# lucidrains/progen

Hardware: NVIDIA H100
Metric: tokens_per_sec (higher is better)
Workload: dtype bf16

## Files before the change

include/progen_b200.h:

```cpp
#ifndef PROGEN_B200_H
#define PROGEN_B200_H
#include <stdint.h>

#ifdef __cplusplus
extern "C" {
#endif

#define PROGEN_F32 0
#define PROGEN_BF16 1

#define PROGEN_BACKEND_SIMT 0
#define PROGEN_BACKEND_TC 1

#define PROGEN_EPI_STORE 0
#define PROGEN_EPI_ROTARY 1
#define PROGEN_EPI_RESIDUAL 2
#define PROGEN_EPI_GLU 3
#define PROGEN_EPI_GELU 4
#define PROGEN_EPI_GLU_BWD 5
#define PROGEN_EPI_GELU_BWD 6
#define PROGEN_EPI_ACCUM 7

const char* progen_version(void);
const char* progen_last_error(void);
// ... 1 lines not shown
long long progen_launch_count(void);

typedef struct progen_gemm_t {
  int32_t M, N, K;
  int32_t a_mn_major, b_mn_major;
  int32_t batch;
  int32_t batch_reduce;
  int32_t causal;
  int32_t split_k;
  int32_t in_dtype, out_dtype, epi_kind, backend;
  int32_t seq_len, dim_head;
  int32_t atomic, tril, tril_rows;
  int64_t lda, ldb;
  int64_t a_batch_rows, b_batch_rows, d_batch_rows;
  int64_t ldo, ldo2, ldaux;
  const void* A;
  const void* B;
  void* out;
  void* out2;
  const float* bias;
  const void* aux;
  const float* rot_sin;
  const float* rot_cos;
} progen_gemm_t;

int progen_gemm(const progen_gemm_t* desc, void* stream);

int progen_embed_fwd(const int* tokens, const float* table, float* x, long long T, int d, int V, void* stream);
int progen_embed_bwd(const int* tokens, const float* dx, float* dtable, long long T, int d, int V, void* stream);

int progen_ln_shift_fwd(const void* x, long long ldx, int x_dtype, const float* scale, void* y, long long ldy, int y_dtype,
                        float* mean, float* rstd, long long T, int d, int seq_len, int shift, void* stream);
int progen_ln_shift_bwd(const void* dy, long long lddy, int act_dtype, const void* x, long long ldx, int x_dtype,
                        const float* scale, const float* mean, const float* rstd, float* dres, void* dout, long long ldo,
                        float* dscale, float* dres_colsum, long long T, int d, int seq_len, int shift, int residual,
                        void* stream);

int progen_colsum(const void* in, long long ld, int dtype, float* out, long long T, int N, void* stream);

int progen_ce_fwd_bwd(const void* logits, int dtype, const int* labels, float* weights, float* loss, void* dlogits,
                      int dlogits_dtype, int B, int n, int V, float inv_batch, void* stream);

int progen_token_logprob(const void* logits, int dtype, const int* labels, float* logp, float* seq_ll, float* seq_count,
                         int B, int n, int V, void* stream);
int progen_preference_head(const void* logits, int dtype, const int* labels, const float* ref_ll, float* logp, float* seq_ll,
                           float* seq_count, float* weights, float* stats, float* loss, float* ce_scratch, void* dlogits,
// ... 124 lines not shown
```

progen_b200/csrc/api.cu:

```cuda
#include <stdarg.h>
#include "gemm.h"
#include "../../include/progen_b200.h"

static thread_local char g_err[1024] = "";
unsigned long long g_progen_launches = 0;

void progen_set_error(const char* fmt, ...) {
  va_list ap;
  va_start(ap, fmt);
  vsnprintf(g_err, sizeof(g_err), fmt, ap);
  va_end(ap);
}

extern "C" {

const char* progen_version(void) { return "progen_b200 0.1.0 (sm_90a; wgmma/TMA GEMM, CUDA " CUDA_VERSION_STR ")"; }

const char* progen_last_error(void) { return g_err; }

long long progen_launch_count(void) { return (long long)__atomic_load_n(&g_progen_launches, __ATOMIC_RELAXED); }

int progen_device_check(void) {
  int dev = 0;
  PG_CUDA(cudaGetDevice(&dev));
// ... 2 lines not shown
  if (prop.major != 9) {
    progen_set_error("device %d (%s) is sm_%d%d; libprogen_b200 is built for sm_90a only", dev, prop.name, prop.major,
                     prop.minor);
    return PROGEN_ERR_DEVICE;
  }
  return PROGEN_OK;
}

int progen_gemm(const progen_gemm_t* d, void* stream) {
  PG_CHECK_ARG(d != nullptr);
  GemmArgs g;
  g.M = d->M; g.N = d->N; g.K = d->K;
  g.A = d->A; g.lda = d->lda; g.a_mn_major = d->a_mn_major;
  g.B = d->B; g.ldb = d->ldb; g.b_mn_major = d->b_mn_major;
  g.batch = d->batch < 1 ? 1 : d->batch;
  g.a_batch_rows = d->a_batch_rows; g.b_batch_rows = d->b_batch_rows; g.d_batch_rows = d->d_batch_rows;
  g.batch_reduce = d->batch_reduce; g.causal = d->causal; g.split_k = d->split_k < 1 ? 1 : d->split_k;
  g.in_dtype = d->in_dtype; g.out_dtype = d->out_dtype; g.epi_kind = d->epi_kind;
  g.epi.out = d->out; g.epi.ldo = d->ldo; g.epi.out2 = d->out2; g.epi.ldo2 = d->ldo2;
  g.epi.bias = d->bias; g.epi.aux = d->aux; g.epi.ldaux = d->ldaux;
  g.epi.rot_sin = d->rot_sin; g.epi.rot_cos = d->rot_cos;
  g.epi.seq_len = d->seq_len > 0 ? d->seq_len : 1; g.epi.dim_head = d->dim_head > 0 ? d->dim_head : 2;
  g.epi.atomic = d->atomic; g.epi.tril = d->tril; g.epi.tril_rows = d->tril_rows > 0 ? d->tril_rows : 1;
  PG_CHECK_ARG(g.epi_kind >= 0 && g.epi_kind < EPI_NUM_KINDS);
  PG_CHECK_ARG(g.epi.out != nullptr);
  if (g.epi_kind == EPI_GLU || g.epi_kind == EPI_GELU) PG_CHECK_ARG(g.epi.bias != nullptr);
  if (g.epi_kind == EPI_GLU_BWD || g.epi_kind == EPI_GELU_BWD) PG_CHECK_ARG(g.epi.aux != nullptr);
  if (g.epi_kind == EPI_ROTARY) PG_CHECK_ARG(g.epi.rot_sin && g.epi.rot_cos && d->seq_len > 0 && d->dim_head > 0 && d->dim_head % 2 == 0);
  if (d->backend == PROGEN_BACKEND_TC) return gemm_tc_launch(g, (cudaStream_t)stream);
  if (d->backend == PROGEN_BACKEND_SIMT) return gemm_simt_launch(g, (cudaStream_t)stream);
  progen_set_error("progen_gemm: unknown backend %d", d->backend);
  return PROGEN_ERR_ARG;
}

}
```

progen_b200/csrc/epilogues.cuh:

```cuda
#pragma once
#include "common.cuh"

enum EpiKind : int {
  EPI_STORE = 0,
  EPI_ROTARY = 1,
  EPI_RESIDUAL = 2,
  EPI_GLU = 3,
  EPI_GELU = 4,
  EPI_GLU_BWD = 5,
  EPI_GELU_BWD = 6,
  EPI_ACCUM = 7,
  EPI_NUM_KINDS = 8
};

struct EpiArgs {
  void* out; long long ldo;
  void* out2; long long ldo2;
  const float* bias;
  const void* aux; long long ldaux;
  const float* rot_sin;
  const float* rot_cos;
  int seq_len; int dim_head;
  int atomic;
  int tril;
  int tril_rows;
};

struct DirectIO {
  template <int N, typename T> __device__ __forceinline__ void store(T* p, long long, const float (&v)[N], bool valid) const {
    if (valid) store_vec<N>(p, v);
  }
  template <int N, typename T> __device__ __forceinline__ void load(const T* p, long long, float (&v)[N], bool valid) const {
    if (valid) load_vec<N>(p, v);
    else {
#pragma unroll
      for (int i = 0; i < N; ++i) v[i] = 0.f;
    }
  }
};

template <int NV> __device__ __forceinline__ void add_bias(const float* __restrict__ bias, int col, float (&v)[NV]) {
#pragma unroll
  for (int i = 0; i < NV; i += 4) {
    const float4 b = __ldg(reinterpret_cast<const float4*>(bias + col + i));
    v[i] += b.x; v[i + 1] += b.y; v[i + 2] += b.z; v[i + 3] += b.w;
  }
}

template <int KIND, typename TO, int NV, typename IO>
__device__ __forceinline__ void epi_apply(const EpiArgs& e, const IO& io, long long row, int col, float (&v)[NV], bool valid) {
  constexpr bool FAST = sizeof(TO) == 2;
  if constexpr (KIND == EPI_STORE) {
    if (e.bias) add_bias<NV>(e.bias, col, v);
    io.template store<NV>(reinterpret_cast<TO*>(e.out) + row * e.ldo + col, e.ldo, v, valid);
  } else if constexpr (KIND == EPI_ROTARY) {
    const int pos = (int)(row % e.seq_len);
    const int half = e.dim_head >> 1;
    const float* sp = e.rot_sin + (long long)pos * half;
    const float* cp = e.rot_cos + (long long)pos * half;
    float o[NV];
    if (e.dim_head % NV == 0) {
      const int j0 = (col % e.dim_head) >> 1;
      float s[NV / 2], c[NV / 2];
      if constexpr (NV >= 32) {
        io.template load<NV / 2>(sp + j0, half, s, true);
        io.template load<NV / 2>(cp + j0, half, c, true);
      } else {
        load_vec<NV / 2>(sp + j0, s);
        load_vec<NV / 2>(cp + j0, c);
      }
#pragma unroll
      for (int i = 0; i < NV; i += 2) {
        o[i] = v[i] * c[i >> 1] - v[i + 1] * s[i >> 1];
        o[i + 1] = v[i + 1] * c[i >> 1] + v[i] * s[i >> 1];
      }
    } else {
#pragma unroll
      for (int i = 0; i < NV; i += 2) {
        const int j = ((col + i) % e.dim_head) >> 1;
        const float s = __ldg(sp + j), c = __ldg(cp + j);
        o[i] = v[i] * c - v[i + 1] * s;
        o[i + 1] = v[i + 1] * c + v[i] * s;
      }
    }
    io.template store<NV>(reinterpret_cast<TO*>(e.out) + row * e.ldo + col, e.ldo, o, valid);
  } else if constexpr (KIND == EPI_RESIDUAL) {
    float* p = reinterpret_cast<float*>(e.out) + row * e.ldo + col;
    float r[NV];
    if (e.aux) io.template load<NV>(reinterpret_cast<const float*>(e.aux) + row * e.ldaux + col, e.ldaux, r, valid);
    else io.template load<NV>(const_cast<const float*>(p), e.ldo, r, valid);
    if (e.bias) add_bias<NV>(e.bias, col, v);
#pragma unroll
    for (int i = 0; i < NV; ++i) r[i] += v[i];
    io.template store<NV>(p, e.ldo, r, valid);
  } else if constexpr (KIND == EPI_GLU) {
    add_bias<NV>(e.bias, col, v);
    if (e.out2) io.template store<NV>(reinterpret_cast<TO*>(e.out2) + row * e.ldo2 + col, e.ldo2, v, valid);
    TO* po = reinterpret_cast<TO*>(e.out) + row * e.ldo + (col >> 1);
    if constexpr (NV >= 16) {
      float o[NV / 2];
#pragma unroll
      for (int i = 0; i < NV / 2; ++i) o[i] = v[2 * i] * gelu_fwd<FAST>(v[2 * i + 1]);
      io.template store<NV / 2>(po, e.ldo, o, valid);
    } else {
      if (valid) {
#pragma unroll
        for (int i = 0; i < NV / 2; ++i) po[i] = from_f32<TO>(v[2 * i] * gelu_fwd<FAST>(v[2 * i + 1]));
      }
    }
  } else if constexpr (KIND == EPI_GELU) {
    add_bias<NV>(e.bias, col, v);
    if (e.out2) io.template store<NV>(reinterpret_cast<TO*>(e.out2) + row * e.ldo2 + col, e.ldo2, v, valid);
    float o[NV];
#pragma unroll
    for (int i = 0; i < NV; ++i) o[i] = gelu_fwd<FAST>(v[i]);
    io.template store<NV>(reinterpret_cast<TO*>(e.out) + row * e.ldo + col, e.ldo, o, valid);
  } else if constexpr (KIND == EPI_GLU_BWD) {
    float u[2 * NV];
    io.template load<2 * NV>(reinterpret_cast<const TO*>(e.aux) + row * e.ldaux + 2 * col, e.ldaux, u, valid);
#pragma unroll
    for (int i = 0; i < NV; ++i) {
      const float dh = v[i], val = u[2 * i], gate = u[2 * i + 1];
      float gf, gd;
      gelu_fwd_bwd<FAST>(gate, gf, gd);
      u[2 * i] = dh * gf;
      u[2 * i + 1] = dh * val * gd;
    }
    io.template store<2 * NV>(reinterpret_cast<TO*>(e.out) + row * e.ldo + 2 * col, e.ldo, u, valid);
  } else if constexpr (KIND == EPI_GELU_BWD) {
    float u[NV];
    io.template load<NV>(reinterpret_cast<const TO*>(e.aux) + row * e.ldaux + col, e.ldaux, u, valid);
#pragma unroll
    for (int i = 0; i < NV; ++i) v[i] *= gelu_bwd<FAST>(u[i]);
    io.template store<NV>(reinterpret_cast<TO*>(e.out) + row * e.ldo + col, e.ldo, v, valid);
  } else if constexpr (KIND == EPI_ACCUM) {
    if (!valid) return;
    float* p = reinterpret_cast<float*>(e.out) + row * e.ldo + col;
    const int lim = e.tril ? (int)(row % e.tril_rows) : 0x7fffffff;
    if (e.atomic) {
#pragma unroll
      for (int i = 0; i < NV; i += 4) {
        if (col + i + 3 <= lim) {
          asm volatile("red.global.add.v4.f32 [%0], {%1, %2, %3, %4};" ::"l"(p + i), "f"(v[i]), "f"(v[i + 1]),
                       "f"(v[i + 2]), "f"(v[i + 3]) : "memory");
        } else {
#pragma unroll
          for (int j = 0; j < 4; ++j)
            if (col + i + j <= lim) atomicAdd(p + i + j, v[i + j]);
        }
      }
    } else {
      float r[NV];
      load_vec<NV>(p, r);
#pragma unroll
      for (int i = 0; i < NV; ++i) r[i] += (col + i <= lim) ? v[i] : 0.f;
      store_vec<NV>(p, r);
    }
  }
}
```

progen_b200/csrc/gemm_simt.cu:

```cuda
#include "gemm.h"

namespace {

constexpr int SBM = 128, SBN = 128, SBK = 16;

struct SimtDev {
  int M, N, K;
  long long a_rs, a_cs, b_rs, b_cs;
  long long a_bs, b_bs;
  long long d_batch_rows;
  int batch_reduce, causal;
  EpiArgs epi;
};

template <typename TI, int KIND, typename TO>
__global__ void __launch_bounds__(256) gemm_simt_kernel(const TI* __restrict__ A, const TI* __restrict__ B, const SimtDev g) {
  __shared__ float As[SBK][SBM + 4];
  __shared__ float Bs[SBK][SBN + 4];
  const int z = blockIdx.z;
  const int m0 = blockIdx.y * SBM, n0 = blockIdx.x * SBN;
  const TI* Ab = A + (long long)z * g.a_bs;
  const TI* Bb = B + (long long)z * g.b_bs;
  const int tid = threadIdx.x;
  const int tx = tid & 15, ty = tid >> 4;
// ... 25 lines not shown
      const int gn = n0 + n, gk = k0 + k;
      Bs[k][n] = (gn < g.N && gk < k_end) ? to_f32(Bb[gn * g.b_rs + gk * g.b_cs]) : 0.f;
    }
    __syncthreads();
#pragma unroll
    for (int k = 0; k < SBK; ++k) {
      float a[8], b[8];
      const float4 a0 = *reinterpret_cast<const float4*>(&As[k][ty * 8]);
      const float4 a1 = *reinterpret_cast<const float4*>(&As[k][ty * 8 + 4]);
      const float4 b0 = *reinterpret_cast<const float4*>(&Bs[k][tx * 8]);
      const float4 b1 = *reinterpret_cast<const float4*>(&Bs[k][tx * 8 + 4]);
      a[0] = a0.x; a[1] = a0.y; a[2] = a0.z; a[3] = a0.w; a[4] = a1.x; a[5] = a1.y; a[6] = a1.z; a[7] = a1.w;
      b[0] = b0.x; b[1] = b0.y; b[2] = b0.z; b[3] = b0.w; b[4] = b1.x; b[5] = b1.y; b[6] = b1.z; b[7] = b1.w;
#pragma unroll
      for (int i = 0; i < 8; ++i)
#pragma unroll
        for (int j = 0; j < 8; ++j) acc[i][j] = fmaf(a[i], b[j], acc[i][j]);
    }
    __syncthreads();
  }

  const int col = n0 + tx * 8;
  if (col >= g.N) return;
#pragma unroll
  for (int i = 0; i < 8; ++i) {
    const int m = m0 + ty * 8 + i;
    if (m >= g.M) break;
    const long long row = (g.batch_reduce ? 0 : (long long)z * g.d_batch_rows) + m;
    epi_apply<KIND, TO, 8>(g.epi, DirectIO{}, row, col, acc[i], true);
  }
}

template <typename TI, int KIND, typename TO>
int launch(const GemmArgs& a, const SimtDev& gd, cudaStream_t stream) {
  dim3 grid((a.N + SBN - 1) / SBN, (a.M + SBM - 1) / SBM, a.batch);
  gemm_simt_kernel<TI, KIND, TO><<<grid, 256, 0, stream>>>(reinterpret_cast<const TI*>(a.A),
                                                          reinterpret_cast<const TI*>(a.B), gd);
  PG_LAUNCH_CHECK();
  return PROGEN_OK;
}

template <typename TI, typename TO>
int dispatch_kind(const GemmArgs& a, const SimtDev& gd, cudaStream_t s) {
  switch (a.epi_kind) {
    case EPI_STORE: return launch<TI, EPI_STORE, TO>(a, gd, s);
    case EPI_ROTARY: return launch<TI, EPI_ROTARY, TO>(a, gd, s);
    case EPI_RESIDUAL: return launch<TI, EPI_RESIDUAL, float>(a, gd, s);
    case EPI_GLU: return launch<TI, EPI_GLU, TO>(a, gd, s);
    case EPI_GELU: return launch<TI, EPI_GELU, TO>(a, gd, s);
    case EPI_GLU_BWD: return launch<TI, EPI_GLU_BWD, TO>(a, gd, s);
    case EPI_GELU_BWD: return launch<TI, EPI_GELU_BWD, TO>(a, gd, s);
    case EPI_ACCUM: return launch<TI, EPI_ACCUM, float>(a, gd, s);
    default: break;
  }
  progen_set_error("gemm_simt: unknown epilogue %d", a.epi_kind);
  return PROGEN_ERR_UNSUPPORTED;
}

}

int gemm_simt_launch(const GemmArgs& a, cudaStream_t stream) {
  PG_CHECK_ARG(a.M > 0 && a.N > 0 && a.K > 0 && a.batch >= 1);
  PG_CHECK_ARG(a.N % 8 == 0);
  PG_CHECK_ARG(a.split_k == 1);
  PG_CHECK_ARG(!a.batch_reduce || (a.epi_kind == EPI_ACCUM && a.epi.atomic));
  SimtDev gd;
  gd.M = a.M; gd.N = a.N; gd.K = a.K;
  gd.a_rs = a.a_mn_major ? 1 : a.lda; gd.a_cs = a.a_mn_major ? a.lda : 1;
  gd.b_rs = a.b_mn_major ? 1 : a.ldb; gd.b_cs = a.b_mn_major ? a.ldb : 1;
  gd.a_bs = a.a_batch_rows * a.lda; gd.b_bs = a.b_batch_rows * a.ldb;
  gd.d_batch_rows = a.d_batch_rows;
  gd.batch_reduce = a.batch_reduce; gd.causal = a.causal;
  gd.epi = a.epi;
  if (a.in_dtype == PG_F32) {
    return dispatch_kind<float, float>(a, gd, stream);
  }
  if (a.out_dtype == PG_BF16) return dispatch_kind<bf16, bf16>(a, gd, stream);
  return dispatch_kind<bf16, float>(a, gd, stream);
}
```

progen_b200/csrc/gemm_tc.cu:

```cuda
#include <cuda.h>
#include <algorithm>
#include <mutex>
#include <unordered_map>
#include "gemm.h"
#include "tc_ptx.cuh"

namespace {

using namespace tc;

constexpr int BM = 128;
constexpr int BN = 128;
constexpr int BK = 64;
constexpr int WG_K = 16;
constexpr int THREADS = 384;
constexpr int A_BYTES = BM * BK * 2;
constexpr int B_BYTES = BN * BK * 2;
constexpr int STAGE_BYTES = A_BYTES + B_BYTES;
constexpr int STAGES = 4;
constexpr int EPI_ROWS = 64;
constexpr int CS_LD = BN + 4;
constexpr int CS_BYTES = EPI_ROWS * CS_LD * 4;
constexpr int SMEM_TOTAL = 1024  + STAGES * STAGE_BYTES + 2 * CS_BYTES + 2 * STAGES * 8;
static_assert(SMEM_TOTAL <= 227 * 1024, "H100: 227 KiB of shared memory per block");
constexpr int BAR_TURN = 1, BAR_EPI = 3;
constexpr int PRODUCER_REGS = 40, CONSUMER_REGS = 232;
static_assert(128 * PRODUCER_REGS + 256 * CONSUMER_REGS <= 65536, "register file");

__device__ __forceinline__ void named_bar_sync(int id, int n) { asm volatile("bar.sync %0, %1;" ::"r"(id), "r"(n) : "memory"); }
__device__ __forceinline__ void named_bar_arrive(int id, int n) { asm volatile("bar.arrive %0, %1;" ::"r"(id), "r"(n) : "memory"); }
template <int R> __device__ __forceinline__ void setmaxnreg_dec() { asm volatile("setmaxnreg.dec.sync.aligned.u32 %0;" ::"n"(R)); }
template <int R> __device__ __forceinline__ void setmaxnreg_inc() { asm volatile("setmaxnreg.inc.sync.aligned.u32 %0;" ::"n"(R)); }

struct GemmDev {
  int M, N, K;
  int batch, batch_reduce;
  int a_batch_rows, b_batch_rows;
  long long d_batch_rows;
  int causal, split_k;
  EpiArgs epi;
};

struct TileInfo {
// ... 109 lines not shown
    for (int kb = ti.kb_begin; kb < ti.kb_end; ++kb) {
      mbar_wait(full_bar(stage), phase);
      const uint32_t sa = smem_base + stage * STAGE_BYTES;
      const uint64_t adesc0 = make_smem_desc<A_MN>(sa), adesc1 = make_smem_desc<A_MN>(sa + 8192);
      const uint64_t bdesc = make_smem_desc<B_MN>(sa + A_BYTES);
      constexpr uint32_t a_step = A_MN ? (2048 >> 4) : (32 >> 4), b_step = B_MN ? (2048 >> 4) : (32 >> 4);
      fence_regs(acc[0]);
      fence_regs(acc[1]);
      wgmma_fence();
#pragma unroll
      for (int k = 0; k < BK / WG_K; ++k) {
        wgmma_m64n128k16_bf16<A_MN ? 1 : 0, B_MN ? 1 : 0>(acc[0], adesc0 + (uint64_t)(k * a_step), bdesc + (uint64_t)(k * b_step));
        wgmma_m64n128k16_bf16<A_MN ? 1 : 0, B_MN ? 1 : 0>(acc[1], adesc1 + (uint64_t)(k * a_step), bdesc + (uint64_t)(k * b_step));
      }
      wgmma_commit();
      fence_regs(acc[0]);
      fence_regs(acc[1]);
      wgmma_wait<1>();
      if (prev >= 0 && tid == 0) mbar_arrive(empty_bar(prev));
      prev = stage;
      advance(1);
    }
    if (t + (int)gridDim.x < tiles) named_bar_arrive(BAR_TURN + (c ^ 1), 256);
    wgmma_wait<0>();
    fence_regs(acc[0]);
    fence_regs(acc[1]);
    if (prev >= 0 && tid == 0) mbar_arrive(empty_bar(prev));

    const int w = tid >> 5, lane = tid & 31;
    const int r0 = 16 * w + (lane >> 2), c0 = 2 * (lane & 3);
#pragma unroll
    for (int h = 0; h < 2; ++h) {
      named_bar_sync(BAR_EPI + c, 128);
#pragma unroll
      for (int j = 0; j < BN / 8; ++j) {
        *reinterpret_cast<float2*>(cs + r0 * CS_LD + 8 * j + c0) = make_float2(acc[h][4 * j], acc[h][4 * j + 1]);
        *reinterpret_cast<float2*>(cs + (r0 + 8) * CS_LD + 8 * j + c0) = make_float2(acc[h][4 * j + 2], acc[h][4 * j + 3]);
      }
      named_bar_sync(BAR_EPI + c, 128);
#pragma unroll 1
      for (int idx = tid; idx < EPI_ROWS * (BN / 8); idx += 128) {
        const int r = idx / (BN / 8), cc = (idx % (BN / 8)) * 8;
        const int m = ti.m0 + EPI_ROWS * h + r, col = ti.n0 + cc;
        if (m >= g.M || col >= g.N) continue;
        float v[8];
        const float4 x0 = *reinterpret_cast<const float4*>(cs + r * CS_LD + cc);
        const float4 x1 = *reinterpret_cast<const float4*>(cs + r * CS_LD + cc + 4);
        v[0] = x0.x; v[1] = x0.y; v[2] = x0.z; v[3] = x0.w; v[4] = x1.x; v[5] = x1.y; v[6] = x1.z; v[7] = x1.w;
        const long long row = (g.batch_reduce ? 0 : (long long)ti.z * g.d_batch_rows) + m;
        epi_apply<KIND, TO, 8>(g.epi, DirectIO{}, row, col, v, true);
      }
    }
  }
}

typedef CUresult (*EncodeTiledFn)(CUtensorMap*, CUtensorMapDataType, cuuint32_t, void*, const cuuint64_t*,
                                  const cuuint64_t*, const cuuint32_t*, const cuuint32_t*, CUtensorMapInterleave,
                                  CUtensorMapSwizzle, CUtensorMapL2promotion, CUtensorMapFloatOOBfill);

EncodeTiledFn get_encode_fn() {
  static EncodeTiledFn fn = nullptr;
  static std::once_flag once;
  std::call_once(once, [] {
    void* p = nullptr;
    cudaDriverEntryPointQueryResult q;
    if (cudaGetDriverEntryPoint("cuTensorMapEncodeTiled", &p, cudaEnableDefault, &q) == cudaSuccess &&
        q == cudaDriverEntryPointSuccess)
      fn = reinterpret_cast<EncodeTiledFn>(p);
  });
  return fn;
}

struct MapKey {
// ... 54 lines not shown
    attr_set = true;
  }
  kern<<<std::min(tiles, pg_num_sms()), THREADS, SMEM_TOTAL, stream>>>(ta, tb, gd, tiles);
  PG_LAUNCH_CHECK();
  return PROGEN_OK;
}

}

int pg_tensor_map_2d_bf16(const void* ptr, uint64_t inner, uint64_t outer, uint64_t row_stride_elems, uint32_t box_inner,
                          uint32_t box_outer, CUtensorMap* out) {
  return get_tensor_map(ptr, inner, outer, row_stride_elems, box_inner, box_outer, out);
}

int gemm_tc_launch(const GemmArgs& a, cudaStream_t stream) {
  PG_CHECK_ARG(a.in_dtype == PG_BF16);
  PG_CHECK_ARG(a.M > 0 && a.N > 0 && a.K > 0 && a.batch >= 1 && a.split_k >= 1);
  PG_CHECK_ARG(a.N % 32 == 0);
  PG_CHECK_ARG(a.K % BK == 0);
  PG_CHECK_ARG(a.lda % 8 == 0 && a.ldb % 8 == 0);
  PG_CHECK_ARG((reinterpret_cast<uintptr_t>(a.A) & 15) == 0 && (reinterpret_cast<uintptr_t>(a.B) & 15) == 0);
  PG_CHECK_ARG(!(a.split_k > 1 && a.causal));
  if (a.epi_kind == EPI_ROTARY) PG_CHECK_ARG(a.epi.seq_len % 32 == 0);
  PG_CHECK_ARG(!(a.split_k > 1 || a.batch_reduce) || (a.epi_kind == EPI_ACCUM && a.epi.atomic));

  const uint64_t a_rows = (a.batch > 1 && a.a_batch_rows > 0) ? (uint64_t)a.a_batch_rows * a.batch
                                                              : (uint64_t)(a.a_mn_major ? a.K : a.M);
  const uint64_t b_rows = (a.batch > 1 && a.b_batch_rows > 0) ? (uint64_t)a.b_batch_rows * a.batch
                                                              : (uint64_t)(a.b_mn_major ? a.K : a.N);
  CUtensorMap ta, tb;
  int rc;
  if (!a.a_mn_major) rc = get_tensor_map(a.A, a.K, a_rows, a.lda, BK, BM, &ta);
  else               rc = get_tensor_map(a.A, a.M, a_rows, a.lda, 64, BK, &ta);
  if (rc) return rc;
  if (!a.b_mn_major) rc = get_tensor_map(a.B, a.K, b_rows, a.ldb, BK, BN, &tb);
  else               rc = get_tensor_map(a.B, a.N, b_rows, a.ldb, 64, BK, &tb);
  if (rc) return rc;

  GemmDev gd;
  gd.M = a.M; gd.N = a.N; gd.K = a.K;
  gd.batch = a.batch; gd.batch_reduce = a.batch_reduce;
  gd.a_batch_rows = (int)a.a_batch_rows; gd.b_batch_rows = (int)a.b_batch_rows; gd.d_batch_rows = a.d_batch_rows;
  gd.causal = a.causal; gd.split_k = a.split_k;
  gd.epi = a.epi;
  const long long tiles = (long long)a.batch * a.split_k * ((a.M + BM - 1) / BM) * ((a.N + BN - 1) / BN);
  PG_CHECK_ARG(tiles < (1ll << 31));
// ... 39 lines not shown
```

progen_b200/engine.py:

```python
import math
import numpy as np
import torch

from . import lib as L

P = 'pro_gen_base/~/'
ALIGN = 64


CUT_ALIGN = 128


def counted_length(labels):
    labels = np.asarray(labels)
    n = labels.shape[1]
    pad = labels == 0
    first = np.where(pad.any(1), pad.argmax(1), n)
    last = np.where((~pad).any(1), n - 1 - (~pad)[:, ::-1].argmax(1), -1)
    return np.minimum(n, np.maximum(first, last) + 1)


def cut_length(labels):
    n = np.asarray(labels).shape[1]
    need = int(counted_length(labels).max()) if len(labels) else 1
# ... 513 lines not shown
                g = f + 'sgu'
                self.wgrad_gemm(s['pj'], half, dres_lp, d, self.G(f + 'linear_1', 'w'))
                self.dgrad_gemm(dres_lp, d, self.W(f + 'linear_1', 'w'), half, self.dpj)
                self.colsum(self.dpj, half, self.G(g + '/~/linear', 'b'))
                self.wgrad_gemm(s['sg'], half, self.dpj, half, self.G(g + '/~/linear', 'w'))
                self.dgrad_gemm(self.dpj, half, self.W(g + '/~/linear', 'w'), half, self.dsg)
                da = self.dh_
                L.check(lib.progen_sgu_gate_bwd(self.dsg.data_ptr(), half, s['hact'].data_ptr(), hid, s['gp'].data_ptr(), half,
                                                self.Pf(g, 'spatial_biases').data_ptr(), da.data_ptr(), hid, self.dgp.data_ptr(),
                                                half, self.G(g, 'spatial_biases').data_ptr(), self.act_dt, T, half, n, st),
                        'sgu_gate_bwd')
                self._mm(M=n, N=n, K=half, A=self.dgp, lda=half, B=s['gn'], ldb=half, out=self.G(g, 'spatial_weights'), ldo=n,
                         epi=L.EPI_ACCUM, out_dtype=L.F32, batch=self.B, a_batch_rows=n, b_batch_rows=n, batch_reduce=True,
                         atomic=True, tril=True, tril_rows=n)
                self._mm(M=n, N=half, K=n, A=self.wm[i], lda=n, a_mn=True, B=self.dgp, ldb=half, b_mn=True, out=self.dgn,
                         ldo=half, out_dtype=self.act_dt, batch=self.B, b_batch_rows=n, d_batch_rows=n, causal=2)
                gate = s['hact'][:, half:]
                L.check(lib.progen_ln_shift_bwd(self.dgn.data_ptr(), half, self.act_dt, gate.data_ptr(), hid, self.act_dt,
                                                self.Pf(g + '/~/layer_norm', 'scale').data_ptr(), s['mean3'].data_ptr(),
                                                s['rstd3'].data_ptr(), 0, da[:, half:].data_ptr(), hid,
                                                self.G(g + '/~/layer_norm', 'scale').data_ptr(), 0, T, half, n, 0, 0, st), 'ln_bwd_sgu')
                L.check(lib.progen_gelu_bwd(da.data_ptr(), s['u'].data_ptr(), self.act_dt, T * hid, st), 'gelu_bwd')
                du, n_in = da, hid
            elif kind == 'glu':
                self.wgrad_gemm(s['hact'], hid, dres_lp, d, self.G(f + 'linear_1', 'w'))
                self.dgrad_gemm(dres_lp, d, self.W(f + 'linear_1', 'w'), hid, self.du, epi=L.EPI_GLU_BWD, ldo=2 * hid,
                                aux=s['u'], ldaux=2 * hid)
                du, n_in = self.du, 2 * hid
            else:
                self.wgrad_gemm(s['hact'], hid, dres_lp, d, self.G(f + 'linear_1', 'w'))
                self.dgrad_gemm(dres_lp, d, self.W(f + 'linear_1', 'w'), hid, self.dh_, epi=L.EPI_GELU_BWD, aux=s['u'], ldaux=hid)
                du, n_in = self.dh_, hid
            self.colsum(du, n_in, self.G(f + 'linear', 'b'))
            self.wgrad_gemm(s['y2'], d, du, n_in, self.G(f + 'linear', 'w'))
            self.dgrad_gemm(du, n_in, self.W(f + 'linear', 'w'), d, self.dy)
            self.ln_bwd_res(self.dy, x1, self.Pf(f + 'layer_norm', 'scale'), s['mean2'], s['rstd2'], self.G(f + 'layer_norm', 'scale'), shift,
                            next_bias_grad=self.G(a + 'linear_1', 'b'))
            self.wgrad_gemm(s['att'], I, dres_lp, d, self.G(a + 'linear_1', 'w'))
            self.dgrad_gemm(dres_lp, d, self.W(a + 'linear_1', 'w'), I, self.datt)
            self.attn_bwd(s['qkv'], s['att'], self.datt, s['lse'], self.dqkv)
            if not self.attn_tc:
                L.check(lib.progen_rotary_bwd(self.dqkv.data_ptr(), 3 * I, self.act_dt, self.rot_sin.data_ptr(),
                                              self.rot_cos.data_ptr(), T, 3 * I, n, self.dh, st), 'rotary_bwd')
            self.wgrad_gemm(s['y1'], d, self.dqkv, 3 * I, self.G(a + 'linear', 'w'))
            self.dgrad_gemm(self.dqkv, 3 * I, self.W(a + 'linear', 'w'), d, self.dy)
            self.ln_bwd_res(self.dy, x0, self.Pf(a + 'layer_norm', 'scale'), s['mean1'], s['rstd1'], self.G(a + 'layer_norm', 'scale'), shift,
                            next_bias_grad=self.G(P + f'ff{i - 1}/~/linear_1', 'b') if i > 0 else None)
            if self.on_layer_grads is not None:
                self.on_layer_grads(i)
        L.check(lib.progen_embed_bwd(self.tok.data_ptr(), self.dres.data_ptr(), self.G(P + 'embed', 'embeddings').data_ptr(),
                                     T, d, self.V, st), 'embed_bwd')
```

progen_b200/lib.py:

```python
import ctypes as C
import os
import torch

F32, BF16 = 0, 1
BACKEND_SIMT, BACKEND_TC = 0, 1
EPI_STORE, EPI_ROTARY, EPI_RESIDUAL, EPI_GLU, EPI_GELU, EPI_GLU_BWD, EPI_GELU_BWD, EPI_ACCUM = range(8)

_HERE = os.path.dirname(os.path.abspath(__file__))
LIB_PATH = os.path.join(_HERE, 'libprogen_b200.so')


class ProgenError(RuntimeError):
    pass


class GemmDesc(C.Structure):
    _fields_ = [
        ('M', C.c_int32), ('N', C.c_int32), ('K', C.c_int32),
        ('a_mn_major', C.c_int32), ('b_mn_major', C.c_int32),
        ('batch', C.c_int32), ('batch_reduce', C.c_int32), ('causal', C.c_int32), ('split_k', C.c_int32),
        ('in_dtype', C.c_int32), ('out_dtype', C.c_int32), ('epi_kind', C.c_int32), ('backend', C.c_int32),
        ('seq_len', C.c_int32), ('dim_head', C.c_int32),
        ('atomic', C.c_int32), ('tril', C.c_int32), ('tril_rows', C.c_int32),
        ('lda', C.c_int64), ('ldb', C.c_int64),
        ('a_batch_rows', C.c_int64), ('b_batch_rows', C.c_int64), ('d_batch_rows', C.c_int64),
        ('ldo', C.c_int64), ('ldo2', C.c_int64), ('ldaux', C.c_int64),
        ('A', C.c_void_p), ('B', C.c_void_p), ('out', C.c_void_p), ('out2', C.c_void_p),
        ('bias', C.c_void_p), ('aux', C.c_void_p), ('rot_sin', C.c_void_p), ('rot_cos', C.c_void_p),
    ]


_lib = None

_LL, _I, _P, _F = C.c_longlong, C.c_int, C.c_void_p, C.c_float

PROTOTYPES = {
    'progen_version': [],
    'progen_last_error': [],
    'progen_device_check': [],
    'progen_launch_count': [],
    'progen_gemm': [C.POINTER(GemmDesc), _P],
    'progen_embed_fwd': [_P, _P, _P, _LL, _I, _I, _P],
    'progen_embed_bwd': [_P, _P, _P, _LL, _I, _I, _P],
    'progen_ln_shift_fwd': [_P, _LL, _I, _P, _P, _LL, _I, _P, _P, _LL, _I, _I, _I, _P],
    'progen_ln_shift_bwd': [_P, _LL, _I, _P, _LL, _I, _P, _P, _P, _P, _P, _LL, _P, _P, _LL, _I, _I, _I, _I, _P],
    'progen_colsum': [_P, _LL, _I, _P, _LL, _I, _P],
    'progen_ce_fwd_bwd': [_P, _I, _P, _P, _P, _P, _I, _I, _I, _I, _F, _P],
    'progen_token_logprob': [_P, _I, _P, _P, _P, _P, _I, _I, _I, _P],
    'progen_preference_head': [_P, _I, _P, _P, _P, _P, _P, _P, _P, _P, _P, _P, _I, _I, _I, _I, _F, _F, _P],
    'progen_masked_mean_pool': [_P, _LL, _I, _P, _P, _I, _I, _I, _P],
    'progen_rotary_bwd': [_P, _LL, _I, _P, _P, _LL, _I, _I, _I, _P],
# ... 46 lines not shown
        raise ProgenError('no CUDA device: progen_b200 has no CPU fallback (sm_90a only)')
    check(load().progen_device_check(), 'progen_device_check')


def dt(t):
    if t.dtype == torch.float32:
        return F32
    if t.dtype == torch.bfloat16:
        return BF16
    raise ProgenError(f'unsupported dtype {t.dtype}')


def ptr(t):
    return 0 if t is None else t.data_ptr()


def stream():
    return torch.cuda.current_stream().cuda_stream


def gemm(*, M, N, K, A, lda, B, ldb, out, ldo, epi=EPI_STORE, backend, a_mn=False, b_mn=False, in_dtype, out_dtype=F32,
         batch=1, a_batch_rows=0, b_batch_rows=0, d_batch_rows=0, batch_reduce=False, causal=0, split_k=1,
         out2=None, ldo2=0, bias=None, aux=None, ldaux=0, rot_sin=None, rot_cos=None, seq_len=0, dim_head=0,
         atomic=False, tril=False, tril_rows=0):
    d = GemmDesc()
    d.M, d.N, d.K = M, N, K
    d.a_mn_major, d.b_mn_major = int(a_mn), int(b_mn)
    d.batch, d.batch_reduce, d.causal, d.split_k = batch, int(batch_reduce), causal, split_k
    d.in_dtype, d.out_dtype, d.epi_kind, d.backend = in_dtype, out_dtype, epi, backend
    d.seq_len, d.dim_head = seq_len, dim_head
    d.atomic, d.tril, d.tril_rows = int(atomic), int(tril), tril_rows
    d.lda, d.ldb = lda, ldb
    d.a_batch_rows, d.b_batch_rows, d.d_batch_rows = a_batch_rows, b_batch_rows, d_batch_rows
    d.ldo, d.ldo2, d.ldaux = ldo, ldo2, ldaux
    as_ptr = lambda x: x if isinstance(x, int) else ptr(x)
    d.A, d.B, d.out, d.out2 = as_ptr(A), as_ptr(B), as_ptr(out), as_ptr(out2)
    d.bias, d.aux, d.rot_sin, d.rot_cos = as_ptr(bias), as_ptr(aux), as_ptr(rot_sin), as_ptr(rot_cos)
    check(load().progen_gemm(C.byref(d), stream()), 'progen_gemm')
```

Before: 970,100.

## Fuse bias-gradient column sums into GEMM backward epilogue and prefetch epilogue operands

Adds an optional colsum output to the GEMM epilogue so the GLU/GELU backward dgrad kernels reduce the feed-forward bias gradient in-kernel, replacing the separate colsum pass over the activation gradient. The TC epilogue is also restructured to prefetch aux, residual and rotary operands into registers before waiting on wgmma, and to load the second half while processing the first. The aim is to remove an extra full read of the gradient tensor and to hide epilogue global-load latency. In exchange it uses more registers, adds shared-memory reductions and atomics per tile, and changes summation order because float atomics are used.

```diff
diff --git a/include/progen_b200.h b/include/progen_b200.h
--- a/include/progen_b200.h
+++ b/include/progen_b200.h
@@ -47,6 +47,7 @@
   const void* aux;
   const float* rot_sin;
   const float* rot_cos;
+  float* colsum;
 } progen_gemm_t;
 
 int progen_gemm(const progen_gemm_t* desc, void* stream);
diff --git a/progen_b200/csrc/api.cu b/progen_b200/csrc/api.cu
--- a/progen_b200/csrc/api.cu
+++ b/progen_b200/csrc/api.cu
@@ -48,8 +48,10 @@
   g.epi.rot_sin = d->rot_sin; g.epi.rot_cos = d->rot_cos;
   g.epi.seq_len = d->seq_len > 0 ? d->seq_len : 1; g.epi.dim_head = d->dim_head > 0 ? d->dim_head : 2;
   g.epi.atomic = d->atomic; g.epi.tril = d->tril; g.epi.tril_rows = d->tril_rows > 0 ? d->tril_rows : 1;
+  g.epi.colsum = d->colsum;
   PG_CHECK_ARG(g.epi_kind >= 0 && g.epi_kind < EPI_NUM_KINDS);
   PG_CHECK_ARG(g.epi.out != nullptr);
+  PG_CHECK_ARG(!g.epi.colsum || g.epi_kind == EPI_GLU_BWD || g.epi_kind == EPI_GELU_BWD);
   if (g.epi_kind == EPI_GLU || g.epi_kind == EPI_GELU) PG_CHECK_ARG(g.epi.bias != nullptr);
   if (g.epi_kind == EPI_GLU_BWD || g.epi_kind == EPI_GELU_BWD) PG_CHECK_ARG(g.epi.aux != nullptr);
   if (g.epi_kind == EPI_ROTARY) PG_CHECK_ARG(g.epi.rot_sin && g.epi.rot_cos && d->seq_len > 0 && d->dim_head > 0 && d->dim_head % 2 == 0);
diff --git a/progen_b200/csrc/epilogues.cuh b/progen_b200/csrc/epilogues.cuh
--- a/progen_b200/csrc/epilogues.cuh
+++ b/progen_b200/csrc/epilogues.cuh
@@ -24,100 +24,162 @@
   int atomic;
   int tril;
   int tril_rows;
-};
-
-struct DirectIO {
-  template <int N, typename T> __device__ __forceinline__ void store(T* p, long long, const float (&v)[N], bool valid) const {
-    if (valid) store_vec<N>(p, v);
-  }
-  template <int N, typename T> __device__ __forceinline__ void load(const T* p, long long, float (&v)[N], bool valid) const {
-    if (valid) load_vec<N>(p, v);
-    else {
-#pragma unroll
-      for (int i = 0; i < N; ++i) v[i] = 0.f;
-    }
-  }
-};
-
-template <int NV> __device__ __forceinline__ void add_bias(const float* __restrict__ bias, int col, float (&v)[NV]) {
-#pragma unroll
-  for (int i = 0; i < NV; i += 4) {
-    const float4 b = __ldg(reinterpret_cast<const float4*>(bias + col + i));
-    v[i] += b.x; v[i + 1] += b.y; v[i + 2] += b.z; v[i + 3] += b.w;
-  }
-}
-
-template <int KIND, typename TO, int NV, typename IO>
-__device__ __forceinline__ void epi_apply(const EpiArgs& e, const IO& io, long long row, int col, float (&v)[NV], bool valid) {
-  constexpr bool FAST = sizeof(TO) == 2;
-  if constexpr (KIND == EPI_STORE) {
-    if (e.bias) add_bias<NV>(e.bias, col, v);
-    io.template store<NV>(reinterpret_cast<TO*>(e.out) + row * e.ldo + col, e.ldo, v, valid);
-  } else if constexpr (KIND == EPI_ROTARY) {
+  float* colsum;
+};
+
+template <int KIND, typename TO, int NV> struct EpiPre {
+  static_assert(NV % 8 == 0, "items are whole 16-byte vectors of bf16 and fp32");
+  static constexpr int BYTES = KIND == EPI_ROTARY ? NV * 4
+                             : KIND == EPI_RESIDUAL ? NV * 4
+                             : KIND == EPI_GLU_BWD ? 2 * NV * (int)sizeof(TO)
+                             : KIND == EPI_GELU_BWD ? NV * (int)sizeof(TO)
+                             : 0;
+  static constexpr int NQ = BYTES / 16;
+  uint4 q[NQ > 0 ? NQ : 1];
+};
+
+template <int NV> struct EpiCol {
+  float b[NV];
+};
+
+template <int KIND, int NV> struct EpiColsum {
+  static constexpr int W = KIND == EPI_GLU_BWD ? 2 * NV : KIND == EPI_GELU_BWD ? NV : 0;
+  static constexpr int REGS = W > 0 ? W : 1;
+  static constexpr int OUT_SCALE = KIND == EPI_GLU_BWD ? 2 : 1;
+};
+
+__device__ __forceinline__ uint4 ld16(const void* p) { return *reinterpret_cast<const uint4*>(p); }
+
+template <typename T, int N> __device__ __forceinline__ void unpack(const uint4* q, float (&v)[N]) {
+  if constexpr (sizeof(T) == 4) {
+#pragma unroll
+    for (int i = 0; i < N / 4; ++i) {
+      v[4 * i] = __uint_as_float(q[i].x); v[4 * i + 1] = __uint_as_float(q[i].y);
+      v[4 * i + 2] = __uint_as_float(q[i].z); v[4 * i + 3] = __uint_as_float(q[i].w);
+    }
+  } else {
+#pragma unroll
+    for (int i = 0; i < N / 8; ++i) {
+      const __nv_bfloat162* h = reinterpret_cast<const __nv_bfloat162*>(&q[i]);
+#pragma unroll
+      for (int j = 0; j < 4; ++j) {
+        const float2 f = __bfloat1622float2(h[j]);
+        v[8 * i + 2 * j] = f.x; v[8 * i + 2 * j + 1] = f.y;
+      }
+    }
+  }
+}
+
+template <int KIND> constexpr bool epi_uses_bias() {
+  return KIND == EPI_STORE || KIND == EPI_RESIDUAL || KIND == EPI_GLU || KIND == EPI_GELU;
+}
+
+template <int KIND, int NV> __device__ __forceinline__ void epi_load_col(const EpiArgs& e, int col, bool valid, EpiCol<NV>& c) {
+  if constexpr (epi_uses_bias<KIND>()) {
+#pragma unroll
+    for (int i = 0; i < NV; i += 4) {
+      const float4 b = (valid && e.bias) ? __ldg(reinterpret_cast<const float4*>(e.bias + col + i)) : make_float4(0.f, 0.f, 0.f, 0.f);
+      c.b[i] = b.x; c.b[i + 1] = b.y; c.b[i + 2] = b.z; c.b[i + 3] = b.w;
+    }
+  }
+}
+
+template <int KIND, typename TO, int NV>
+__device__ __forceinline__ void epi_load(const EpiArgs& e, long long row, int col, bool valid, EpiPre<KIND, TO, NV>& p) {
+  constexpr int NQ = EpiPre<KIND, TO, NV>::NQ;
+  if constexpr (NQ > 0) {
+    if (!valid) {
+#pragma unroll
+      for (int i = 0; i < NQ; ++i) p.q[i] = make_uint4(0u, 0u, 0u, 0u);
+      return;
+    }
+  }
+  if constexpr (KIND == EPI_ROTARY) {
     const int pos = (int)(row % e.seq_len);
     const int half = e.dim_head >> 1;
     const float* sp = e.rot_sin + (long long)pos * half;
     const float* cp = e.rot_cos + (long long)pos * half;
-    float o[NV];
     if (e.dim_head % NV == 0) {
       const int j0 = (col % e.dim_head) >> 1;
-      float s[NV / 2], c[NV / 2];
-      if constexpr (NV >= 32) {
-        io.template load<NV / 2>(sp + j0, half, s, true);
-        io.template load<NV / 2>(cp + j0, half, c, true);
-      } else {
-        load_vec<NV / 2>(sp + j0, s);
-        load_vec<NV / 2>(cp + j0, c);
-      }
-#pragma unroll
-      for (int i = 0; i < NV; i += 2) {
-        o[i] = v[i] * c[i >> 1] - v[i + 1] * s[i >> 1];
-        o[i + 1] = v[i + 1] * c[i >> 1] + v[i] * s[i >> 1];
+#pragma unroll
+      for (int i = 0; i < NQ / 2; ++i) {
+        p.q[i] = ld16(sp + j0 + 4 * i);
+        p.q[NQ / 2 + i] = ld16(cp + j0 + 4 * i);
       }
     } else {
+      uint32_t s[NV / 2], c[NV / 2];
 #pragma unroll
       for (int i = 0; i < NV; i += 2) {
         const int j = ((col + i) % e.dim_head) >> 1;
-        const float s = __ldg(sp + j), c = __ldg(cp + j);
-        o[i] = v[i] * c - v[i + 1] * s;
-        o[i + 1] = v[i + 1] * c + v[i] * s;
-      }
-    }
-    io.template store<NV>(reinterpret_cast<TO*>(e.out) + row * e.ldo + col, e.ldo, o, valid);
+        s[i >> 1] = __float_as_uint(__ldg(sp + j));
+        c[i >> 1] = __float_as_uint(__ldg(cp + j));
+      }
+#pragma unroll
+      for (int i = 0; i < NQ / 2; ++i) {
+        p.q[i] = make_uint4(s[4 * i], s[4 * i + 1], s[4 * i + 2], s[4 * i + 3]);
+        p.q[NQ / 2 + i] = make_uint4(c[4 * i], c[4 * i + 1], c[4 * i + 2], c[4 * i + 3]);
+      }
+    }
   } else if constexpr (KIND == EPI_RESIDUAL) {
-    float* p = reinterpret_cast<float*>(e.out) + row * e.ldo + col;
+    const float* r = e.aux ? reinterpret_cast<const float*>(e.aux) + row * e.ldaux + col
+                           : reinterpret_cast<const float*>(e.out) + row * e.ldo + col;
+#pragma unroll
+    for (int i = 0; i < NQ; ++i) p.q[i] = ld16(r + 4 * i);
+  } else if constexpr (KIND == EPI_GLU_BWD) {
+    const TO* u = reinterpret_cast<const TO*>(e.aux) + row * e.ldaux + 2 * col;
+#pragma unroll
+    for (int i = 0; i < NQ; ++i) p.q[i] = ld16(reinterpret_cast<const uint8_t*>(u) + 16 * i);
+  } else if constexpr (KIND == EPI_GELU_BWD) {
+    const TO* u = reinterpret_cast<const TO*>(e.aux) + row * e.ldaux + col;
+#pragma unroll
+    for (int i = 0; i < NQ; ++i) p.q[i] = ld16(reinterpret_cast<const uint8_t*>(u) + 16 * i);
+  }
+}
+
+template <int KIND, typename TO, int NV, int CW>
+__device__ __forceinline__ void epi_finish(const EpiArgs& e, long long row, int col, float (&v)[NV], const EpiCol<NV>& cb,
+                                           const EpiPre<KIND, TO, NV>& p, bool valid, float (&csum)[CW]) {
+  constexpr bool FAST = sizeof(TO) == 2;
+  if constexpr (epi_uses_bias<KIND>()) {
+    if (KIND == EPI_GLU || KIND == EPI_GELU || e.bias) {
+#pragma unroll
+      for (int i = 0; i < NV; ++i) v[i] += cb.b[i];
+    }
+  }
+  if constexpr (KIND == EPI_STORE) {
+    if (valid) store_vec<NV>(reinterpret_cast<TO*>(e.out) + row * e.ldo + col, v);
+  } else if constexpr (KIND == EPI_ROTARY) {
+    float s[NV / 2], c[NV / 2], o[NV];
+    unpack<float>(&p.q[0], s);
+    unpack<float>(&p.q[EpiPre<KIND, TO, NV>::NQ / 2], c);
+#pragma unroll
+    for (int i = 0; i < NV; i += 2) {
+      o[i] = v[i] * c[i >> 1] - v[i + 1] * s[i >> 1];
+      o[i + 1] = v[i + 1] * c[i >> 1] + v[i] * s[i >> 1];
+    }
+    if (valid) store_vec<NV>(reinterpret_cast<TO*>(e.out) + row * e.ldo + col, o);
+  } else if constexpr (KIND == EPI_RESIDUAL) {
     float r[NV];
-    if (e.aux) io.template load<NV>(reinterpret_cast<const float*>(e.aux) + row * e.ldaux + col, e.ldaux, r, valid);
-    else io.template load<NV>(const_cast<const float*>(p), e.ldo, r, valid);
-    if (e.bias) add_bias<NV>(e.bias, col, v);
+    unpack<float>(p.q, r);
 #pragma unroll
     for (int i = 0; i < NV; ++i) r[i] += v[i];
-    io.template store<NV>(p, e.ldo, r, valid);
+    if (valid) store_vec<NV>(reinterpret_cast<float*>(e.out) + row * e.ldo + col, r);
   } else if constexpr (KIND == EPI_GLU) {
-    add_bias<NV>(e.bias, col, v);
-    if (e.out2) io.template store<NV>(reinterpret_cast<TO*>(e.out2) + row * e.ldo2 + col, e.ldo2, v, valid);
+    if (e.out2 && valid) store_vec<NV>(reinterpret_cast<TO*>(e.out2) + row * e.ldo2 + col, v);
     TO* po = reinterpret_cast<TO*>(e.out) + row * e.ldo + (col >> 1);
-    if constexpr (NV >= 16) {
-      float o[NV / 2];
-#pragma unroll
-      for (int i = 0; i < NV / 2; ++i) o[i] = v[2 * i] * gelu_fwd<FAST>(v[2 * i + 1]);
-      io.template store<NV / 2>(po, e.ldo, o, valid);
-    } else {
-      if (valid) {
-#pragma unroll
-        for (int i = 0; i < NV / 2; ++i) po[i] = from_f32<TO>(v[2 * i] * gelu_fwd<FAST>(v[2 * i + 1]));
-      }
+    if (valid) {
+#pragma unroll
+      for (int i = 0; i < NV / 2; ++i) po[i] = from_f32<TO>(v[2 * i] * gelu_fwd<FAST>(v[2 * i + 1]));
     }
   } else if constexpr (KIND == EPI_GELU) {
-    add_bias<NV>(e.bias, col, v);
-    if (e.out2) io.template store<NV>(reinterpret_cast<TO*>(e.out2) + row * e.ldo2 + col, e.ldo2, v, valid);
+    if (e.out2 && valid) store_vec<NV>(reinterpret_cast<TO*>(e.out2) + row * e.ldo2 + col, v);
     float o[NV];
 #pragma unroll
     for (int i = 0; i < NV; ++i) o[i] = gelu_fwd<FAST>(v[i]);
-    io.template store<NV>(reinterpret_cast<TO*>(e.out) + row * e.ldo + col, e.ldo, o, valid);
+    if (valid) store_vec<NV>(reinterpret_cast<TO*>(e.out) + row * e.ldo + col, o);
   } else if constexpr (KIND == EPI_GLU_BWD) {
     float u[2 * NV];
-    io.template load<2 * NV>(reinterpret_cast<const TO*>(e.aux) + row * e.ldaux + 2 * col, e.ldaux, u, valid);
+    unpack<TO>(p.q, u);
 #pragma unroll
     for (int i = 0; i < NV; ++i) {
       const float dh = v[i], val = u[2 * i], gate = u[2 * i + 1];
@@ -126,35 +188,47 @@
       u[2 * i] = dh * gf;
       u[2 * i + 1] = dh * val * gd;
     }
-    io.template store<2 * NV>(reinterpret_cast<TO*>(e.out) + row * e.ldo + 2 * col, e.ldo, u, valid);
+    if (valid) {
+      store_vec<2 * NV>(reinterpret_cast<TO*>(e.out) + row * e.ldo + 2 * col, u);
+      if (e.colsum) {
+#pragma unroll
+        for (int i = 0; i < 2 * NV; ++i) csum[i] += to_f32(from_f32<TO>(u[i]));
+      }
+    }
   } else if constexpr (KIND == EPI_GELU_BWD) {
     float u[NV];
-    io.template load<NV>(reinterpret_cast<const TO*>(e.aux) + row * e.ldaux + col, e.ldaux, u, valid);
+    unpack<TO>(p.q, u);
 #pragma unroll
     for (int i = 0; i < NV; ++i) v[i] *= gelu_bwd<FAST>(u[i]);
-    io.template store<NV>(reinterpret_cast<TO*>(e.out) + row * e.ldo + col, e.ldo, v, valid);
+    if (valid) {
+      store_vec<NV>(reinterpret_cast<TO*>(e.out) + row * e.ldo + col, v);
+      if (e.colsum) {
+#pragma unroll
+        for (int i = 0; i < NV; ++i) csum[i] += to_f32(from_f32<TO>(v[i]));
+      }
+    }
   } else if constexpr (KIND == EPI_ACCUM) {
     if (!valid) return;
-    float* p = reinterpret_cast<float*>(e.out) + row * e.ldo + col;
+    float* po = reinterpret_cast<float*>(e.out) + row * e.ldo + col;
     const int lim = e.tril ? (int)(row % e.tril_rows) : 0x7fffffff;
     if (e.atomic) {
 #pragma unroll
       for (int i = 0; i < NV; i += 4) {
         if (col + i + 3 <= lim) {
-          asm volatile("red.global.add.v4.f32 [%0], {%1, %2, %3, %4};" ::"l"(p + i), "f"(v[i]), "f"(v[i + 1]),
+          asm volatile("red.global.add.v4.f32 [%0], {%1, %2, %3, %4};" ::"l"(po + i), "f"(v[i]), "f"(v[i + 1]),
                        "f"(v[i + 2]), "f"(v[i + 3]) : "memory");
         } else {
 #pragma unroll
           for (int j = 0; j < 4; ++j)
-            if (col + i + j <= lim) atomicAdd(p + i + j, v[i + j]);
+            if (col + i + j <= lim) atomicAdd(po + i + j, v[i + j]);
         }
       }
     } else {
       float r[NV];
-      load_vec<NV>(p, r);
+      load_vec<NV>(po, r);
 #pragma unroll
       for (int i = 0; i < NV; ++i) r[i] += (col + i <= lim) ? v[i] : 0.f;
-      store_vec<NV>(p, r);
-    }
-  }
-}
+      store_vec<NV>(po, r);
+    }
+  }
+}
diff --git a/progen_b200/csrc/gemm_simt.cu b/progen_b200/csrc/gemm_simt.cu
--- a/progen_b200/csrc/gemm_simt.cu
+++ b/progen_b200/csrc/gemm_simt.cu
@@ -71,12 +71,26 @@
 
   const int col = n0 + tx * 8;
   if (col >= g.N) return;
+  using CS = EpiColsum<KIND, 8>;
+  EpiCol<8> cb;
+  epi_load_col<KIND, 8>(g.epi, col, true, cb);
+  float csum[CS::REGS];
+#pragma unroll
+  for (int k = 0; k < CS::REGS; ++k) csum[k] = 0.f;
 #pragma unroll
   for (int i = 0; i < 8; ++i) {
     const int m = m0 + ty * 8 + i;
     if (m >= g.M) break;
     const long long row = (g.batch_reduce ? 0 : (long long)z * g.d_batch_rows) + m;
-    epi_apply<KIND, TO, 8>(g.epi, DirectIO{}, row, col, acc[i], true);
+    EpiPre<KIND, TO, 8> pre;
+    epi_load<KIND, TO, 8>(g.epi, row, col, true, pre);
+    epi_finish<KIND, TO, 8>(g.epi, row, col, acc[i], cb, pre, true, csum);
+  }
+  if constexpr (CS::W > 0) {
+    if (g.epi.colsum) {
+#pragma unroll
+      for (int k = 0; k < CS::W; ++k) atomicAdd(g.epi.colsum + CS::OUT_SCALE * col + k, csum[k]);
+    }
   }
 }
 
@@ -112,8 +126,7 @@
   PG_CHECK_ARG(a.M > 0 && a.N > 0 && a.K > 0 && a.batch >= 1);
   PG_CHECK_ARG(a.N % 8 == 0);
   PG_CHECK_ARG(a.split_k == 1);
-  PG_CHECK_ARG(!a.batch_reduce || (a.epi_kind == EPI_ACCUM && a.epi.atomic));
-  SimtDev gd;
+  PG_CHECK_ARG(!a.batch_reduce || (a.epi_kind == EPI_ACCUM && a.epi.atomic));  SimtDev gd;
   gd.M = a.M; gd.N = a.N; gd.K = a.K;
   gd.a_rs = a.a_mn_major ? 1 : a.lda; gd.a_cs = a.a_mn_major ? a.lda : 1;
   gd.b_rs = a.b_mn_major ? 1 : a.ldb; gd.b_cs = a.b_mn_major ? a.ldb : 1;
diff --git a/progen_b200/csrc/gemm_tc.cu b/progen_b200/csrc/gemm_tc.cu
--- a/progen_b200/csrc/gemm_tc.cu
+++ b/progen_b200/csrc/gemm_tc.cu
@@ -19,6 +19,7 @@
 constexpr int STAGE_BYTES = A_BYTES + B_BYTES;
 constexpr int STAGES = 4;
 constexpr int EPI_ROWS = 64;
+constexpr int EPI_ITEMS = EPI_ROWS * (BN / 8) / 128;
 constexpr int CS_LD = BN + 4;
 constexpr int CS_BYTES = EPI_ROWS * CS_LD * 4;
 constexpr int SMEM_TOTAL = 1024  + STAGES * STAGE_BYTES + 2 * CS_BYTES + 2 * STAGES * 8;
@@ -174,13 +175,32 @@
       advance(1);
     }
     if (t + (int)gridDim.x < tiles) named_bar_arrive(BAR_TURN + (c ^ 1), 256);
+
+    const int w = tid >> 5, lane = tid & 31;
+    const int r0 = 16 * w + (lane >> 2), c0 = 2 * (lane & 3);
+    const int cc = 8 * (tid & 15), col = ti.n0 + cc;
+    const bool col_ok = col < g.N;
+    const int m_first = ti.m0 + (tid >> 4);
+    const long long row_first = (g.batch_reduce ? 0 : (long long)ti.z * g.d_batch_rows) + m_first;
+    using CS = EpiColsum<KIND, 8>;
+    EpiCol<8> cb;
+    EpiPre<KIND, TO, 8> pre[EPI_ITEMS];
+    epi_load_col<KIND, 8>(g.epi, col, col_ok, cb);
+    constexpr bool LOAD_BEFORE_WAIT = KIND != EPI_RESIDUAL;
+    auto load_pass0 = [&] {
+#pragma unroll
+      for (int i = 0; i < EPI_ITEMS; ++i)
+        epi_load<KIND, TO, 8>(g.epi, row_first + 8 * i, col, col_ok && m_first + 8 * i < g.M, pre[i]);
+    };
+    if constexpr (LOAD_BEFORE_WAIT) load_pass0();
     wgmma_wait<0>();
     fence_regs(acc[0]);
     fence_regs(acc[1]);
     if (prev >= 0 && tid == 0) mbar_arrive(empty_bar(prev));
 
-    const int w = tid >> 5, lane = tid & 31;
-    const int r0 = 16 * w + (lane >> 2), c0 = 2 * (lane & 3);
+    float csum[CS::REGS];
+#pragma unroll
+    for (int k = 0; k < CS::REGS; ++k) csum[k] = 0.f;
 #pragma unroll
     for (int h = 0; h < 2; ++h) {
       named_bar_sync(BAR_EPI + c, 128);
@@ -189,18 +209,48 @@
         *reinterpret_cast<float2*>(cs + r0 * CS_LD + 8 * j + c0) = make_float2(acc[h][4 * j], acc[h][4 * j + 1]);
         *reinterpret_cast<float2*>(cs + (r0 + 8) * CS_LD + 8 * j + c0) = make_float2(acc[h][4 * j + 2], acc[h][4 * j + 3]);
       }
+      if constexpr (!LOAD_BEFORE_WAIT) {
+        if (h == 0) load_pass0();
+      }
       named_bar_sync(BAR_EPI + c, 128);
-#pragma unroll 1
-      for (int idx = tid; idx < EPI_ROWS * (BN / 8); idx += 128) {
-        const int r = idx / (BN / 8), cc = (idx % (BN / 8)) * 8;
-        const int m = ti.m0 + EPI_ROWS * h + r, col = ti.n0 + cc;
-        if (m >= g.M || col >= g.N) continue;
+#pragma unroll
+      for (int i = 0; i < EPI_ITEMS; ++i) {
+        const int r = 8 * i + (tid >> 4);
+        const int m = m_first + EPI_ROWS * h + 8 * i;
         float v[8];
         const float4 x0 = *reinterpret_cast<const float4*>(cs + r * CS_LD + cc);
         const float4 x1 = *reinterpret_cast<const float4*>(cs + r * CS_LD + cc + 4);
         v[0] = x0.x; v[1] = x0.y; v[2] = x0.z; v[3] = x0.w; v[4] = x1.x; v[5] = x1.y; v[6] = x1.z; v[7] = x1.w;
-        const long long row = (g.batch_reduce ? 0 : (long long)ti.z * g.d_batch_rows) + m;
-        epi_apply<KIND, TO, 8>(g.epi, DirectIO{}, row, col, v, true);
+        epi_finish<KIND, TO, 8>(g.epi, row_first + EPI_ROWS * h + 8 * i, col, v, cb, pre[i], col_ok && m < g.M, csum);
+        if (h == 0)
+          epi_load<KIND, TO, 8>(g.epi, row_first + EPI_ROWS + 8 * i, col, col_ok && m + EPI_ROWS < g.M, pre[i]);
+      }
+    }
+    if constexpr (CS::W > 0) {
+      if (g.epi.colsum) {
+        constexpr int TW = 16 * CS::W;
+#pragma unroll
+        for (int k = 0; k < CS::W; ++k) csum[k] += __shfl_xor_sync(0xffffffffu, csum[k], 16);
+        named_bar_sync(BAR_EPI + c, 128);
+        if (lane < 16) {
+#pragma unroll
+          for (int k = 0; k < CS::W; k += 4)
+            *reinterpret_cast<float4*>(cs + w * TW + lane * CS::W + k) = make_float4(csum[k], csum[k + 1], csum[k + 2], csum[k + 3]);
+        }
+        named_bar_sync(BAR_EPI + c, 128);
+        const int out0 = CS::OUT_SCALE * ti.n0, out_cols = CS::OUT_SCALE * g.N;
+#pragma unroll
+        for (int q = tid; q < TW / 4; q += 128) {
+          float4 s = *reinterpret_cast<const float4*>(cs + 4 * q);
+#pragma unroll
+          for (int ww = 1; ww < 4; ++ww) {
+            const float4 x = *reinterpret_cast<const float4*>(cs + ww * TW + 4 * q);
+            s.x += x.x; s.y += x.y; s.z += x.z; s.w += x.w;
+          }
+          if (out0 + 4 * q < out_cols)
+            asm volatile("red.global.add.v4.f32 [%0], {%1, %2, %3, %4};" ::"l"(g.epi.colsum + out0 + 4 * q), "f"(s.x),
+                         "f"(s.y), "f"(s.z), "f"(s.w) : "memory");
+        }
       }
     }
   }
@@ -301,6 +351,7 @@
   PG_CHECK_ARG((reinterpret_cast<uintptr_t>(a.A) & 15) == 0 && (reinterpret_cast<uintptr_t>(a.B) & 15) == 0);
   PG_CHECK_ARG(!(a.split_k > 1 && a.causal));
   if (a.epi_kind == EPI_ROTARY) PG_CHECK_ARG(a.epi.seq_len % 32 == 0);
+  PG_CHECK_ARG((reinterpret_cast<uintptr_t>(a.epi.colsum) & 15) == 0);
   PG_CHECK_ARG(!(a.split_k > 1 || a.batch_reduce) || (a.epi_kind == EPI_ACCUM && a.epi.atomic));
 
   const uint64_t a_rows = (a.batch > 1 && a.a_batch_rows > 0) ? (uint64_t)a.a_batch_rows * a.batch
diff --git a/progen_b200/engine.py b/progen_b200/engine.py
--- a/progen_b200/engine.py
+++ b/progen_b200/engine.py
@@ -559,16 +559,17 @@
                                                 self.G(g + '/~/layer_norm', 'scale').data_ptr(), 0, T, half, n, 0, 0, st), 'ln_bwd_sgu')
                 L.check(lib.progen_gelu_bwd(da.data_ptr(), s['u'].data_ptr(), self.act_dt, T * hid, st), 'gelu_bwd')
                 du, n_in = da, hid
+                self.colsum(du, n_in, self.G(f + 'linear', 'b'))
             elif kind == 'glu':
                 self.wgrad_gemm(s['hact'], hid, dres_lp, d, self.G(f + 'linear_1', 'w'))
                 self.dgrad_gemm(dres_lp, d, self.W(f + 'linear_1', 'w'), hid, self.du, epi=L.EPI_GLU_BWD, ldo=2 * hid,
-                                aux=s['u'], ldaux=2 * hid)
+                                aux=s['u'], ldaux=2 * hid, colsum=self.G(f + 'linear', 'b'))
                 du, n_in = self.du, 2 * hid
             else:
                 self.wgrad_gemm(s['hact'], hid, dres_lp, d, self.G(f + 'linear_1', 'w'))
-                self.dgrad_gemm(dres_lp, d, self.W(f + 'linear_1', 'w'), hid, self.dh_, epi=L.EPI_GELU_BWD, aux=s['u'], ldaux=hid)
+                self.dgrad_gemm(dres_lp, d, self.W(f + 'linear_1', 'w'), hid, self.dh_, epi=L.EPI_GELU_BWD, aux=s['u'], ldaux=hid,
+                                colsum=self.G(f + 'linear', 'b'))
                 du, n_in = self.dh_, hid
-            self.colsum(du, n_in, self.G(f + 'linear', 'b'))
             self.wgrad_gemm(s['y2'], d, du, n_in, self.G(f + 'linear', 'w'))
             self.dgrad_gemm(du, n_in, self.W(f + 'linear', 'w'), d, self.dy)
             self.ln_bwd_res(self.dy, x1, self.Pf(f + 'layer_norm', 'scale'), s['mean2'], s['rstd2'], self.G(f + 'layer_norm', 'scale'), shift,
diff --git a/progen_b200/lib.py b/progen_b200/lib.py
--- a/progen_b200/lib.py
+++ b/progen_b200/lib.py
@@ -27,6 +27,7 @@
         ('ldo', C.c_int64), ('ldo2', C.c_int64), ('ldaux', C.c_int64),
         ('A', C.c_void_p), ('B', C.c_void_p), ('out', C.c_void_p), ('out2', C.c_void_p),
         ('bias', C.c_void_p), ('aux', C.c_void_p), ('rot_sin', C.c_void_p), ('rot_cos', C.c_void_p),
+        ('colsum', C.c_void_p),
     ]
 
 
@@ -119,7 +120,7 @@
 def gemm(*, M, N, K, A, lda, B, ldb, out, ldo, epi=EPI_STORE, backend, a_mn=False, b_mn=False, in_dtype, out_dtype=F32,
          batch=1, a_batch_rows=0, b_batch_rows=0, d_batch_rows=0, batch_reduce=False, causal=0, split_k=1,
          out2=None, ldo2=0, bias=None, aux=None, ldaux=0, rot_sin=None, rot_cos=None, seq_len=0, dim_head=0,
-         atomic=False, tril=False, tril_rows=0):
+         atomic=False, tril=False, tril_rows=0, colsum=None):
     d = GemmDesc()
     d.M, d.N, d.K = M, N, K
     d.a_mn_major, d.b_mn_major = int(a_mn), int(b_mn)
@@ -133,4 +134,5 @@
     as_ptr = lambda x: x if isinstance(x, int) else ptr(x)
     d.A, d.B, d.out, d.out2 = as_ptr(A), as_ptr(B), as_ptr(out), as_ptr(out2)
     d.bias, d.aux, d.rot_sin, d.rot_cos = as_ptr(bias), as_ptr(aux), as_ptr(rot_sin), as_ptr(rot_cos)
+    d.colsum = as_ptr(colsum)
     check(load().progen_gemm(C.byref(d), stream()), 'progen_gemm')
```

Result: faster. 1.032 million (median of 6 runs) (+6.3%).
